# foolwood/SiamMask

Hardware: NVIDIA H100
Metric: search-region frames/sec (127/255 SiamMask-sharp) (higher is better)
Workload: dtype f16x3 (hi+lo split fp16 operands on wgmma, f32 accumulate; f32 CUDA-core xcorr/refine)

## Files before the change

siammask_b200/csrc/common.cuh:

```cuda
#pragma once
#include <cuda.h>
#include <cuda_fp16.h>
#include <cuda_runtime.h>
#include <cstdint>
#include <cstdio>
#include <stdexcept>
#include <string>
#include <vector>

struct sm_image_desc;

namespace smk {

struct Act {
  __half* hi = nullptr;
  __half* lo = nullptr;
  int B = 0, H = 0, W = 0, C = 0;
  int sexp = 0;
  __host__ __device__ size_t numel() const { return (size_t)B * H * W * C; }
  __host__ __device__ int M() const { return B * H * W; }
};

struct ConvGeom {
  int Cin, Cout, KH, KW, stride, pad, dil;
// ... 8 lines not shown
  const __half* res_hi = nullptr;
  const __half* res_lo = nullptr;
  __half* out_hi = nullptr;
  __half* out_lo = nullptr;
  float* out_f32 = nullptr;
  int out_mode = OUT_NHWC_SPLIT;
  int relu = 0;
  int* ovf = nullptr;
};

__device__ __forceinline__ void flag_if_out_of_range(float absmax, int* ovf) {
  if (ovf != nullptr && !(absmax <= 65504.f)) atomicOr(ovf, 1);
}
constexpr int kStatusBadSlot = 2;

struct GemmSegment {
  CUtensorMap tmA[2];
  int kind;
  int mode;
  int num_kb, cblks, KW;
  int stride, pad, dil;
  int b_col0;
};

struct GemmParams {
  GemmSegment seg[2];
  int nseg;
  CUtensorMap tmB[2];
  int M, Cout, Ho, Wo;
  int n_tiles, m_tiles;
  int reverse_m;
  Epilogue ep;
};

struct GemmInput {
  Act in;
  ConvGeom g;
  int w_col0;
};

struct TrackerHp {
  double context_amount, penalty_k, window_influence, lr;
  int32_t exemplar_size, instance_size, total_stride, base_size, out_size, reserved;
};

struct CudaError : std::runtime_error {
  using std::runtime_error::runtime_error;
};

#define SMK_CUDA(expr)                                                                              \
  do {                                                                                              \
    cudaError_t _e = (expr);                                                                        \
    if (_e != cudaSuccess)                                                                          \
      throw smk::CudaError(std::string(#expr) + " failed: " + cudaGetErrorString(_e) + " at " +    \
                           __FILE__ + ":" + std::to_string(__LINE__));                              \
  } while (0)

#define SMK_CHECK(cond, msg)                                                                        \
  do {                                                                                              \
    if (!(cond)) throw std::runtime_error(std::string("check failed: ") + #cond + " — " + (msg));   \
  } while (0)

template <typename K>
inline void ensure_dynamic_smem(K kernel, int bytes, unsigned long long& done_mask) {
  int dev = 0;
  SMK_CUDA(cudaGetDevice(&dev));
  const unsigned long long bit = 1ull << (dev & 63);
  if (done_mask & bit) return;
  SMK_CUDA(cudaFuncSetAttribute(kernel, cudaFuncAttributeMaxDynamicSharedMemorySize, bytes));
  done_mask |= bit;
}


bool gemm_conv_supported(const ConvGeom& g);
void launch_gemm_conv(const Act& in, const ConvGeom& g, const __half* w_hi, const __half* w_lo, int cout_pad,
                      const Epilogue& ep, int nsplit, int num_sms, cudaStream_t st);
void launch_gemm_multi(const GemmInput* convs, int nconv, const Act* residual, int res_col0, const __half* w_hi,
                       const __half* w_lo, int cout_pad, int w_ld, const Epilogue& ep, int nsplit, int num_sms,
                       cudaStream_t st, bool reverse_m = false);

CUtensorMap make_map_tiled_nd(const __half* base, int rank, const uint64_t* dims, const uint64_t* strides_bytes,
                              const uint32_t* box, int swizzle_bytes);

bool patch_conv_supported(const Act& in, const ConvGeom& g);
void launch_conv3x3_patch(const Act& in, const ConvGeom& g, const __half* w_hi, const __half* w_lo, int w_ld,
                          const Epilogue& ep, int nsplit, int num_sms, cudaStream_t st);

void launch_stem_tc(const float* x_nchw, int B, int S, const __half* w_hi, const __half* w_lo, const float* alpha,
                    const float* beta, Act out, int num_sms, cudaStream_t st, int* ovf = nullptr);

void launch_ref_conv(const Act& in, const ConvGeom& g, const float* w_krsc_cout, const Epilogue& ep,
                     cudaStream_t st);
void launch_stem(const float* x_nchw, int B, int S, const float* w, const float* alpha, const float* beta, Act out,
                 cudaStream_t st);
void launch_maxpool3s2(const Act& in, Act out, cudaStream_t st);
void launch_xcorr_nhwc(const Act& x, int c_off, const __half* k_hi, const __half* k_lo, int kh, int kw, Act out,
                       float mul, int* ovf, cudaStream_t st, const int32_t* slots = nullptr, int num_slots = 0);
void launch_scatter_slots(const __half* src_hi, const __half* src_lo, __half* dst_hi, __half* dst_lo,
                          const int32_t* slots, int B, int num_slots, int n, int* status, cudaStream_t st);
void launch_paste_labels(const float* masks, int side, const double* maps, const uint8_t* anno, const int32_t* obj_off,
                         const int32_t* objects, int G, int H, int W, double seg_thr, uint8_t* labels, cudaStream_t st,
                         const sm_image_desc* desc = nullptr);
void launch_paste_labels_iou(const float* masks, int side, const double* maps, const uint8_t* anno,
                             const int32_t* obj_off, const int32_t* objects, const int32_t* target_ids, int G, int H,
                             int W, double seg_thr, uint8_t* labels, const double* thrs, int T, int32_t* counts,
                             cudaStream_t st, const sm_image_desc* desc = nullptr);
void launch_label_boxes(const uint8_t* anno, int G, int H, int W, const int32_t* queries, int Q, int32_t* boxes,
                        cudaStream_t st, const sm_image_desc* desc = nullptr);
void launch_vot_overlap(const float* poly_a, const float* poly_b, int B, int W, int H, float* overlap, cudaStream_t st,
                        const int32_t* wh = nullptr);
void launch_absmax(const Act& a, float* slot, cudaStream_t st);
void launch_xcorr_nchw_f32(const float* x, const float* k, float* out, int planes, int H, int W, int kh, int kw,
                           cudaStream_t st);
int launch_xcorr_bulk_f32(const float* x, const float* k, float* out, int planes, int H, int W, int kh, int kw,
                          cudaStream_t st);
void launch_crop_center(const Act& in, int crop, Act out, cudaStream_t st);
void launch_refine_crop(const Act& in, const int32_t* pos, int pos_max, int scale, int padv, int size, Act out,
                        cudaStream_t st);
void launch_gather_corr(const Act& corr, const int32_t* pos, float* out, float mul, cudaStream_t st);
void launch_gather_mask_col(const float* mask, const int32_t* pos, int B, int C, int R, float* out, cudaStream_t st);
void launch_deconv(const float* p3, const float* w, const float* bias, float* out, int B, int Cin, int N,
                   int cout, cudaStream_t st);
void launch_split_to_f32(const Act& in, float* out, cudaStream_t st, float mul = 1.f);
void launch_import_nchw(const float* x_nchw, Act out, cudaStream_t st);
void launch_warp_affine(const float* src, int sh, int sw, const double* maps, float* dst, int dh, int dw, float border,
                        int B, cudaStream_t st, const sm_image_desc* dst_desc = nullptr);
void launch_tracker_prepare(int B, const double* state, const int32_t* avg, const TrackerHp& hp, int32_t* boxes,
                            double* tsz, double* aux, cudaStream_t st);
void launch_tracker_update(int B, double* state, const float* rec, const double* aux, const int32_t* imsize,
                           const TrackerHp& hp, int A, int R, double* maps, double* out, cudaStream_t st,
                           const double* hp_table = nullptr);
void launch_crop_resize(const uint8_t* frames, size_t frame_stride, int H, int W, const int32_t* box, int B, int model,
                        float* out, cudaStream_t st, const int32_t* frame_idx = nullptr,
                        const sm_image_desc* desc = nullptr);
void launch_select(const float* cls, const float* loc, const float* anchors, const float* window, const double* tsz,
                   int B, int A, int R, double penalty_k, double window_influence, int32_t* best_idx, int32_t* pos,
                   float* rec, cudaStream_t st, const double* hp = nullptr);
void launch_mask_iou(const float* masks, int side, const double* maps, const uint8_t* anno, const int32_t* video, int B,
                     int H, int W, const double* thrs, int T, int32_t* counts, cudaStream_t st);
void launch_small_conv3x3_maps(const float* a, const float* b, int B, int Hi, int Wi, int Ho, int Wo, int Cin, int Cout,
                               const int* ymap, const int* xmap, const float* w, const float* bias, int relu,
                               float* out, cudaStream_t st);
std::vector<int> nearest_index_table(int out_size, int in_size);
int gemm_cout_pad(int cout);

}
```

siammask_b200/csrc/conv3x3_patch_sm90.cu:

```cuda
#include "common.cuh"
#include "ptx.cuh"

#include <cstdlib>

namespace smk {

namespace {

constexpr int P_THREADS = 384;
constexpr int P_CONSUMER_WARPS = 8;
constexpr int P_SLACK_ROWS = 8;

template <int CM, int NSPLIT>
struct PCfg {
  static constexpr int NKB = CM / 64;
  static constexpr int B_TILE_BYTES = CM * 128;
  static constexpr int B_STAGE_BYTES = NSPLIT * B_TILE_BYTES;
  static constexpr int B_STAGES = 3;
  static constexpr int ACC = CM / 2;
};

struct PatchParams {
  CUtensorMap tmA[2];
  CUtensorMap tmB[2];
  int B, H, W, PW, RO;
  int tiles_per_img, num_tiles;
  int panel_bytes;
  int patch_rows;
  Epilogue ep;
};

__device__ __forceinline__ void tma_load_4d(void* dst, const CUtensorMap* map, uint64_t* bar, int c0, int c1, int c2,
                                            int c3) {
  asm volatile(
      "cp.async.bulk.tensor.4d.shared::cluster.global.mbarrier::complete_tx::bytes"
      " [%0], [%1, {%3, %4, %5, %6}], [%2];" ::"r"(smem_u32(dst)),
      "l"(reinterpret_cast<uint64_t>(map)), "r"(smem_u32(bar)), "r"(c0), "r"(c1), "r"(c2), "r"(c3)
      : "memory");
}

template <int CM, int NSPLIT>
__global__ void __launch_bounds__(P_THREADS, 1) conv3x3_patch_kernel(const __grid_constant__ PatchParams p) {
  using C = PCfg<CM, NSPLIT>;
  constexpr int NKB = C::NKB;
  extern __shared__ uint8_t smem_raw[];
  uint8_t* smem = reinterpret_cast<uint8_t*>((reinterpret_cast<uintptr_t>(smem_raw) + 1023) & ~uintptr_t(1023));
  const int patch_bytes = NSPLIT * p.panel_bytes;
  uint8_t* bring = smem + 2 * patch_bytes;
  uint64_t* pfull = reinterpret_cast<uint64_t*>(bring + C::B_STAGES * C::B_STAGE_BYTES);
  uint64_t* pempty = pfull + 2;
  uint64_t* bfull = pempty + 2;
  uint64_t* bempty = bfull + C::B_STAGES;

  const int warp = __shfl_sync(0xffffffffu, (int)(threadIdx.x >> 5), 0), lane = threadIdx.x & 31;
  const int slack_bytes = P_SLACK_ROWS * 128;
  for (int pb = 0; pb < 2 * NSPLIT; ++pb) {
    uint8_t* panel = smem + pb * p.panel_bytes;
    for (int i = threadIdx.x * 16; i < 2 * slack_bytes; i += P_THREADS * 16) {
      uint8_t* dst = i < slack_bytes ? panel + i : panel + slack_bytes + p.patch_rows * 128 + (i - slack_bytes);
      *reinterpret_cast<uint4*>(dst) = make_uint4(0, 0, 0, 0);
    }
  }
  fence_proxy_async();
  if (threadIdx.x == 0) {
    for (int i = 0; i < NSPLIT; ++i) { tma_prefetch_desc(&p.tmA[i]); tma_prefetch_desc(&p.tmB[i]); }
    for (int i = 0; i < 2; ++i) { mbar_init(&pfull[i], 1); mbar_init(&pempty[i], P_CONSUMER_WARPS); }
    for (int i = 0; i < C::B_STAGES; ++i) { mbar_init(&bfull[i], 1); mbar_init(&bempty[i], P_CONSUMER_WARPS); }
    fence_barrier_init();
  }
  __syncthreads();

  if (warp < 4) {
    setmaxnreg_dec<40>();
    if (warp != 0) return;
    const bool leader = elect_one();
    const int my_tiles = (p.num_tiles - (int)blockIdx.x + (int)gridDim.x - 1) / (int)gridDim.x;
    const int units = my_tiles * NKB;
    auto issue_patch = [&](int u) {
      const int tile = blockIdx.x + (u / NKB) * gridDim.x;
      const int kb = u % NKB;
      const int b = tile / p.tiles_per_img;
      const int y0 = (tile - b * p.tiles_per_img) * p.RO;
      const int pbuf = u & 1;
      const uint32_t pph = (u >> 1) & 1;
      mbar_wait(&pempty[pbuf], pph ^ 1);
      if (leader) {
        mbar_arrive_expect_tx(&pfull[pbuf], NSPLIT * p.patch_rows * 128);
#pragma unroll
        for (int s = 0; s < NSPLIT; ++s)
          tma_load_4d(smem + (pbuf * NSPLIT + s) * p.panel_bytes + slack_bytes, &p.tmA[s], &pfull[pbuf], kb * 64, -1,
                      y0 - 1, b);
      }
      __syncwarp();
    };
    int bstage = 0;
    uint32_t bphase = 0;
    if (units > 0) issue_patch(0);
    for (int u = 0; u < units; ++u) {
      const int kb = u % NKB;
      for (int tap = 0; tap < 9; ++tap) {
        if (tap == C::B_STAGES && u + 1 < units) issue_patch(u + 1);
        mbar_wait(&bempty[bstage], bphase ^ 1);
        if (leader) {
          mbar_arrive_expect_tx(&bfull[bstage], C::B_STAGE_BYTES);
          uint8_t* st = bring + bstage * C::B_STAGE_BYTES;
#pragma unroll
          for (int s = 0; s < NSPLIT; ++s)
            tma_load_2d(st + s * C::B_TILE_BYTES, &p.tmB[s], &bfull[bstage], tap * CM + kb * 64, 0);
        }
        __syncwarp();
        if (++bstage == C::B_STAGES) { bstage = 0; bphase ^= 1; }
      }
    }
    return;
  }

  setmaxnreg_inc<232>();
  const int wg = (warp >> 2) - 1;
  const int wl = warp & 3;
  const Epilogue& ep = p.ep;
  float acc[C::ACC];
  float acc2[C::ACC];
  int unit = 0, bstage = 0;
  uint32_t bphase = 0;
  for (int tile = blockIdx.x; tile < p.num_tiles; tile += gridDim.x) {
#pragma unroll
    for (int i = 0; i < C::ACC; ++i) { acc[i] = 0.f; acc2[i] = 0.f; }
    for (int kb = 0; kb < NKB; ++kb, ++unit) {
      const int pbuf = unit & 1;
      const uint32_t pph = (unit >> 1) & 1;
      mbar_wait(&pfull[pbuf], pph);
      const uint32_t a_hi0 = smem_u32(smem + (pbuf * NSPLIT) * p.panel_bytes + slack_bytes) + wg * (64 * 128);
      const uint32_t a_lo0 = a_hi0 + p.panel_bytes;
      int prev = -1;
#pragma unroll 1
      for (int tap = 0; tap < 9; ++tap) {
        const int r = tap / 3, s = tap - 3 * r;
        const int shift = (r * p.PW + s - 1) * 128;
        mbar_wait(&bfull[bstage], bphase);
        const uint32_t b_hi = smem_u32(bring + bstage * C::B_STAGE_BYTES);
        const uint64_t da_hi = wgmma_desc_kmajor<128>(a_hi0 + shift);
        const uint64_t da_lo = wgmma_desc_kmajor<128>(a_lo0 + shift);
        const uint64_t db_hi = wgmma_desc_kmajor<128>(b_hi);
        const uint64_t db_lo = wgmma_desc_kmajor<128>(b_hi + C::B_TILE_BYTES);
        wgmma_fence();
#pragma unroll
        for (int k = 0; k < 4; ++k) {
          const uint64_t kadd = static_cast<uint64_t>(k * 2);
          wgmma_f16<CM>(acc, da_hi + kadd, db_hi + kadd);
          if constexpr (NSPLIT == 2) {
            wgmma_f16<CM>(acc2, da_hi + kadd, db_lo + kadd);
            wgmma_f16<CM>(acc2, da_lo + kadd, db_hi + kadd);
          }
        }
        wgmma_commit();
        wgmma_wait<1>();
        if (prev >= 0) {
          __syncwarp();
          if (lane == 0) mbar_arrive(&bempty[prev]);
        }
        prev = bstage;
        if (++bstage == C::B_STAGES) { bstage = 0; bphase ^= 1; }
      }
      wgmma_wait<0>();
      __syncwarp();
      if (lane == 0) {
        mbar_arrive(&bempty[prev]);
        mbar_arrive(&pempty[pbuf]);
      }
    }
    fence_regs(acc);
    if constexpr (NSPLIT == 2) fence_regs(acc2);

    const int b = tile / p.tiles_per_img;
    const int y0 = (tile - b * p.tiles_per_img) * p.RO;
    const int j0 = wg * 64 + wl * 16 + (lane >> 2);
    float amax = 0.f;
#pragma unroll
    for (int h = 0; h < 2; ++h) {
      const int j = j0 + 8 * h;
      const int yy = j / p.PW, xx = j - yy * p.PW;
      const int y = y0 + yy, x = xx - 1;
      if (!(x >= 0 && x < p.W && y < p.H && yy < p.RO)) continue;
      const size_t off0 = ((static_cast<size_t>(b) * p.H + y) * p.W + x) * CM;
#pragma unroll
      for (int q = 0; q < CM / 8; ++q) {
        const int n = 8 * q + 2 * (lane & 3);
        float v0 = acc[4 * q + 2 * h], v1 = acc[4 * q + 2 * h + 1];
        if constexpr (NSPLIT == 2) {
          v0 += acc2[4 * q + 2 * h];
          v1 += acc2[4 * q + 2 * h + 1];
        }
        const float2 al = __ldg(reinterpret_cast<const float2*>(ep.alpha + n));
        const float2 be = __ldg(reinterpret_cast<const float2*>(ep.beta + n));
        v0 = fmaf(v0, al.x, be.x);
        v1 = fmaf(v1, al.y, be.y);
        if (ep.relu) {
          v0 = fmaxf(v0, 0.f);
          v1 = fmaxf(v1, 0.f);
        }
        amax = fmaxf(amax, fmaxf(fabsf(v0), fabsf(v1)));
        const __half2 hv = __floats2half2_rn(v0, v1);
        const float2 hf = __half22float2(hv);
        *reinterpret_cast<__half2*>(ep.out_hi + off0 + n) = hv;
        if (ep.out_lo != nullptr)
          *reinterpret_cast<__half2*>(ep.out_lo + off0 + n) = __floats2half2_rn(v0 - hf.x, v1 - hf.y);
      }
    }
    flag_if_out_of_range(amax, ep.ovf);
  }
}

int patch_pw(int W) { return (W + 1 + 7) / 8 * 8; }

int patch_ro(int W) {
  const int pw = patch_pw(W);
  return 128 % pw == 0 ? 128 / pw : 0;
}

template <int CM, int NSPLIT>
void launch_patch(const PatchParams& p, int num_sms, cudaStream_t st) {
  using C = PCfg<CM, NSPLIT>;
  const int smem = 2 * NSPLIT * p.panel_bytes + C::B_STAGES * C::B_STAGE_BYTES + 256 + 1024;
  SMK_CHECK(smem <= 227 * 1024, "patch conv: shared memory budget");
  auto kern = conv3x3_patch_kernel<CM, NSPLIT>;
  static unsigned long long attr = 0;
  ensure_dynamic_smem(kern, 227 * 1024, attr);
  const int grid = p.num_tiles < num_sms ? p.num_tiles : num_sms;
  kern<<<grid, P_THREADS, smem, st>>>(p);
  SMK_CUDA(cudaGetLastError());
}

}

bool patch_conv_supported(const Act& in, const ConvGeom& g) {
  if (!(g.KH == 3 && g.KW == 3 && g.stride == 1 && g.pad == 1 && g.dil == 1 && g.Cin == g.Cout)) return false;
  if (!(g.Cin == 64 || g.Cin == 128)) return false;
  if (in.H != in.W) return false;
  return patch_ro(in.W) >= 1 && patch_pw(in.W) <= 64;
}

void launch_conv3x3_patch(const Act& in, const ConvGeom& g, const __half* w_hi, const __half* w_lo, int w_ld,
                          const Epilogue& ep, int nsplit, int num_sms, cudaStream_t st) {
  SMK_CHECK(patch_conv_supported(in, g), "patch conv: unsupported geometry");
  SMK_CHECK(ep.out_mode == OUT_NHWC_SPLIT && ep.res_hi == nullptr, "patch conv writes NHWC split planes, no residual");
  SMK_CHECK(nsplit == 1 || (in.lo != nullptr && w_lo != nullptr && ep.out_lo != nullptr), "exact mode needs lo planes");
  SMK_CHECK(w_ld >= 9 * g.Cin, "weight row length");
  PatchParams p;
  p.B = in.B; p.H = in.H; p.W = in.W;
  p.PW = patch_pw(in.W);
  p.RO = patch_ro(in.W);
  p.tiles_per_img = (in.H + p.RO - 1) / p.RO;
  p.num_tiles = in.B * p.tiles_per_img;
  p.patch_rows = (p.RO + 2) * p.PW;
  p.panel_bytes = (p.patch_rows + 2 * P_SLACK_ROWS) * 128;
  SMK_CHECK(p.panel_bytes % 1024 == 0, "patch panels must keep the 1024-byte swizzle alignment");
  p.ep = ep;
  for (int s = 0; s < nsplit; ++s) {
    const __half* a = s == 0 ? in.hi : in.lo;
    const uint64_t dims[4] = {(uint64_t)in.C, (uint64_t)in.W, (uint64_t)in.H, (uint64_t)in.B};
    const uint64_t strides[3] = {(uint64_t)in.C * 2, (uint64_t)in.W * in.C * 2, (uint64_t)in.H * in.W * in.C * 2};
    const uint32_t box[4] = {64, (uint32_t)p.PW, (uint32_t)(p.RO + 2), 1};
    p.tmA[s] = make_map_tiled_nd(a, 4, dims, strides, box, 128);
    const uint64_t wd[2] = {(uint64_t)w_ld, (uint64_t)g.Cout};
    const uint64_t ws[1] = {(uint64_t)w_ld * 2};
    const uint32_t wb[2] = {64, (uint32_t)g.Cout};
    p.tmB[s] = make_map_tiled_nd(s == 0 ? w_hi : w_lo, 2, wd, ws, wb, 128);
  }
  if (nsplit == 1) { p.tmA[1] = p.tmA[0]; p.tmB[1] = p.tmB[0]; }
  if (g.Cin == 64) {
    if (nsplit == 2) launch_patch<64, 2>(p, num_sms, st); else launch_patch<64, 1>(p, num_sms, st);
  } else {
    if (nsplit == 2) launch_patch<128, 2>(p, num_sms, st); else launch_patch<128, 1>(p, num_sms, st);
  }
}

}
```

siammask_b200/csrc/engine.cu:

```cuda
#include "../../include/siammask_b200.h"
#include "common.cuh"

#include <algorithm>
#include <cmath>
#include <cstdlib>
#include <cstring>
#include <map>
#include <memory>
#include <unordered_map>

namespace smk {

namespace {

constexpr float BN_EPS = 1e-5f;
constexpr size_t ALIGN = 256;
inline size_t align_up(size_t x) { return (x + ALIGN - 1) / ALIGN * ALIGN; }

thread_local std::string g_last_error;

struct ConvW {
  ConvGeom g{};
  int cout_pad = 0;
  bool gemm_ok = false;
// ... 879 lines not shown
        const int step = !(mx[i] <= 65504.f) ? -10 : (mx[i] == 0.f && iter < 8) ? +10 : 0;
        if (step != 0) set_scale(absmax_names_[i], std::max(-60, std::min(60, scale_of(absmax_names_[i]) + step)));
      }
      rewire_and_upload();
      continue;
    }
    settled = true;
    for (size_t i = 0; i < mx.size(); ++i) {
      if (mx[i] == 0.f) continue;
      const int cur = scale_of(absmax_names_[i]);
      if (mx[i] >= 256.f && mx[i] <= 4096.f) continue;
      int want = cur + (int)std::lround(std::log2(1024.0 / (double)mx[i]));
      want = std::max(-60, std::min(60, want));
      const auto it = layers_.find(absmax_names_[i]);
      if (it != layers_.end() && it->second.f32_out) want = 0;
      if (want != cur) { set_scale(absmax_names_[i], want); settled = false; }
    }
    if (!settled) rewire_and_upload();
  }
  SMK_CHECK(settled, "calibrate(): activation scales did not settle (non-finite network outputs?)");
}

int Engine::status() {
  int v = 0;
  SMK_CUDA(cudaDeviceSynchronize());
  SMK_CUDA(cudaMemcpy(&v, ovf_flag_, sizeof(int), cudaMemcpyDeviceToHost));
  return v;
}


Act Engine::alloc_act(Arena& ar, int B, int H, int W, int C) {
  Act a;
  a.B = B; a.H = H; a.W = W; a.C = C;
  a.hi = static_cast<__half*>(ar.alloc(a.numel() * sizeof(__half)));
  a.lo = exact_ ? static_cast<__half*>(ar.alloc(a.numel() * sizeof(__half))) : nullptr;
  return a;
}

F32T Engine::alloc_f32(Arena& ar, int B, int H, int W, int C) {
  F32T t;
  t.B = B; t.H = H; t.W = W; t.C = C;
  t.p = static_cast<float*>(ar.alloc((size_t)B * H * W * C * sizeof(float)));
  return t;
}

void Engine::conv_into(const Act& in, const ConvW& Lw, Epilogue ep, cudaStream_t st, const Act* res,
                       const Act* in2) {
  ep.beta = Lw.beta;
  const double M = (double)in.B * Lw.g.out_size(in.H) * Lw.g.out_size(in.W);
  double K = (double)Lw.g.KH * Lw.g.KW * Lw.g.Cin;
  const bool tc = cfg_.backend == SM_BACKEND_TENSOR && Lw.gemm_ok;
  SMK_CHECK(in2 == nullptr || (tc && Lw.fused2), "fused second input needs the tensor-core path");
  if (in2 != nullptr) K += (double)Lw.g2.KH * Lw.g2.KW * Lw.g2.Cin;
  if (calibrating_) {
    ConvW& W = const_cast<ConvW&>(Lw);
    auto name_of = [&](const Act& a) {
      auto it = tensor_name_.find(a.hi);
      return it == tensor_name_.end() ? std::string() : it->second;
    };
    W.src_in = name_of(in);
    W.src_in2 = in2 ? name_of(*in2) : std::string();
    W.src_res = res ? name_of(*res) : std::string();
    W.f32_out = ep.out_mode != OUT_NHWC_SPLIT;
  }
  SMK_CHECK(in.sexp == Lw.s_in && (in2 == nullptr || in2->sexp == Lw.s_in2) && (res == nullptr || res->sexp == Lw.s_res),
            "activation scale mismatch at " + Lw.conv_key + " (weights were packed for other scales: re-run calibrate)");
  SMK_CHECK(ep.out_mode == OUT_NHWC_SPLIT || Lw.s_out == 0, "fp32 outputs are unscaled");
  if (ep.out_mode == OUT_NHWC_SPLIT) ep.ovf = ovf_flag_;
  const double flops = 2.0 * M * K * Lw.g.Cout;
  const double bytes = 4.0 * ((double)in.numel() + (in2 ? (double)in2->numel() : 0.0) + M * Lw.g.Cout * (res ? 2 : 1) +
                              K * Lw.g.Cout);
  if (!tc) {
    SMK_CHECK(Lw.s_in == 0 && Lw.s_out == 0, "the SIMT backend runs unscaled activations only");
    ep.alpha = ones_;
    if (res != nullptr) { ep.res_hi = res->hi; ep.res_lo = res->lo; }
    launch(st, 1, Lw.conv_key, "conv_simt", flops, bytes, [&] { launch_ref_conv(in, Lw.g, Lw.w_ref, ep, st); });
    return;
  }
  ep.alpha = Lw.alpha;
  const Act* big = &in;
  if (in2 != nullptr && in2->numel() > big->numel()) big = in2;
  if (res != nullptr && res->numel() > big->numel()) big = res;
  const bool use_patch = in2 == nullptr && res == nullptr && ep.out_mode == OUT_NHWC_SPLIT &&
                         patch_conv_supported(in, Lw.g);
  const bool reverse = !use_patch && end_of(*big) > 0;
  GemmInput gi[2] = {{in, Lw.g, 0}, {in, Lw.g, 0}};
  int nconv = 1;
  const Act* ident = nullptr;
  if (in2 != nullptr) {
    gi[1] = {*in2, Lw.g2, Lw.col2};
    nconv = 2;
    ep.beta = Lw.beta2;
  } else if (res != nullptr) {
    if (Lw.has_diag) ident = res;
    else { ep.res_hi = res->hi; ep.res_lo = res->lo; }
  }
  launch(st, 1, Lw.conv_key, "conv_gemm", flops, bytes, [&] {
    const int now_end = reverse ? -1 : +1;
    last_end_[in.hi] = now_end;
    if (in2 != nullptr) last_end_[in2->hi] = now_end;
    if (res != nullptr) last_end_[res->hi] = now_end;
    if (ep.out_mode == OUT_NHWC_SPLIT) last_end_[ep.out_hi] = now_end;
    if (use_patch)
      launch_conv3x3_patch(in, Lw.g, Lw.w_hi, Lw.w_lo, Lw.w_ld, ep, exact_ ? 2 : 1, num_sms_, st);
    else
      launch_gemm_multi(gi, nconv, ident, Lw.col_diag, Lw.w_hi, Lw.w_lo, Lw.cout_pad, Lw.w_ld, ep, exact_ ? 2 : 1,
                        num_sms_, st, reverse);
  });
}

void Engine::note_tensor(const Act& a, const std::string& name, cudaStream_t st, const Act* same_scale_as) {
  if (measuring_) return;
  if (taps_ != nullptr) (*taps_)[name] = a;
  if (!calibrating_) return;
  if (same_scale_as != nullptr) {
    tensor_name_[a.hi] = tensor_name_[same_scale_as->hi];
    return;
  }
  tensor_name_[a.hi] = name;
  size_t slot = 0;
  for (; slot < absmax_names_.size(); ++slot)
    if (absmax_names_[slot] == name) break;
  if (slot == absmax_names_.size()) {
    SMK_CHECK((int)slot < kAbsmaxSlots, "too many calibrated tensors");
    absmax_names_.push_back(name);
  }
  launch_absmax(a, absmax_dev_ + slot, st);
}

void Engine::note_tensor(const F32T& t, const std::string& name) {
  if (!measuring_ && taps_f32_ != nullptr) (*taps_f32_)[name] = t;
}

Act Engine::conv(const Act& in, const ConvW& Lw, bool relu, const Act* res, Arena& ar, cudaStream_t st,
                 const Act* in2) {
  Act out = alloc_act(ar, in.B, Lw.g.out_size(in.H), Lw.g.out_size(in.W), Lw.g.Cout);
  Epilogue ep;
  ep.relu = relu ? 1 : 0;
  ep.out_mode = OUT_NHWC_SPLIT;
  ep.out_hi = out.hi;
  ep.out_lo = out.lo;
  out.sexp = Lw.s_out;
  conv_into(in, Lw, ep, st, res, in2);
  note_tensor(out, Lw.conv_key, st);
  return out;
}

F32T Engine::conv_f32(const Act& in, const ConvW& Lw, bool relu, Arena& ar, cudaStream_t st) {
  F32T out = alloc_f32(ar, in.B, Lw.g.out_size(in.H), Lw.g.out_size(in.W), Lw.g.Cout);
  Epilogue ep;
  ep.relu = relu ? 1 : 0;
  ep.out_mode = OUT_NHWC_F32;
  ep.out_f32 = out.p;
  conv_into(in, Lw, ep, st);
  note_tensor(out, Lw.conv_key);
  return out;
}

Act Engine::backbone(const float* x, int B, int S, Arena& ar, std::map<std::string, Act>* keep, cudaStream_t st) {
  const std::string F = "features.features.";
  const int So = (S - 7) / 2 + 1;
  Act p0 = alloc_act(ar, B, So, So, 64);
  const ConvW& stem = L(F + "conv1");
  launch(st, 1, "stem", "stem", 2.0 * B * So * So * 64 * 147, 4.0 * B * (3.0 * S * S + 64.0 * So * So), [&] {
    if (cfg_.backend == SM_BACKEND_TENSOR)
      launch_stem_tc(x, B, S, stem_whi_, stem_wlo_, stem_alpha_, stem.beta, p0, num_sms_, st, ovf_flag_);
    else launch_stem(x, B, S, stem.w_ref, ones_, stem.beta, p0, st);
// ... 509 lines not shown
  SMK_CUDA(cudaDeviceSynchronize());
  std::string out;
  for (auto& r : prof_) {
    float ms = 0.f;
    cudaEventElapsedTime(&ms, r.e0, r.e1);
    char line[512];
    snprintf(line, sizeof line, "%s\t%s\t%.6f\t%.0f\t%.0f\n", r.name.c_str(), r.cat.c_str(), ms, r.flops, r.bytes);
    out += line;
    event_pool_.push_back(r.e0);
    event_pool_.push_back(r.e1);
  }
  prof_.clear();
  return out;
}


static void conv2d_op(const float* x, const float* w, const float* scale, const float* shift, float* out, int B,
                      int Cin, int H, int W, int Cout, int KH, int KW, int stride, int pad, int dil, int relu,
                      int backend, int precision, cudaStream_t st) {
  ConvGeom g{Cin, Cout, KH, KW, stride, pad, dil};
  const bool exact = precision == SM_PRECISION_EXACT;
  const bool use_gemm = backend == SM_BACKEND_TENSOR;
  SMK_CHECK(!use_gemm || gemm_conv_supported(g), "tensor-core conv needs Cin % 64 == 0");
  const size_t K = (size_t)KH * KW * Cin;
  const int cout_pad = use_gemm ? gemm_cout_pad(Cout) : Cout;
  std::vector<float> hw(K * Cout), hs(Cout, 1.f), hb(Cout, 0.f);
  SMK_CUDA(cudaStreamSynchronize(st));
  SMK_CUDA(cudaMemcpy(hw.data(), w, hw.size() * sizeof(float), cudaMemcpyDeviceToHost));
  if (scale) SMK_CUDA(cudaMemcpy(hs.data(), scale, Cout * sizeof(float), cudaMemcpyDeviceToHost));
  if (shift) SMK_CUDA(cudaMemcpy(hb.data(), shift, Cout * sizeof(float), cudaMemcpyDeviceToHost));
  std::vector<float> wref(K * Cout), alpha(cout_pad, 0.f), beta(cout_pad, 0.f);
  std::vector<__half> whi((size_t)cout_pad * K, __float2half_rn(0.f)), wlo((size_t)cout_pad * K, __float2half_rn(0.f));
  const int HW = KH * KW;
  for (int n = 0; n < Cout; ++n) {
    float amax = 0.f;
    for (int c = 0; c < Cin; ++c)
      for (int t = 0; t < HW; ++t) {
        const float fw = (float)((double)hw[((size_t)n * Cin + c) * HW + t] * (double)hs[n]);
        wref[((size_t)t * Cin + c) * Cout + n] = fw;
        amax = std::max(amax, std::fabs(fw));
      }
    beta[n] = hb[n];
    alpha[n] = 1.f;
    if (use_gemm) {
      const int e = weight_exp(amax);
      alpha[n] = std::ldexp(1.f, -e);
      for (int c = 0; c < Cin; ++c)
        for (int t = 0; t < HW; ++t) {
          const float fw = std::ldexp(wref[((size_t)t * Cin + c) * Cout + n], e);
          const __half h = __float2half_rn(fw);
          whi[((size_t)n * HW + t) * Cin + c] = h;
          wlo[((size_t)n * HW + t) * Cin + c] = __float2half_rn(fw - __half2float(h));
        }
    }
  }
  const int Ho = g.out_size(H), Wo = g.out_size(W);
  Act in;
  in.B = B; in.H = H; in.W = W; in.C = Cin;
  __half *d_whi = nullptr, *d_wlo = nullptr;
  float *d_wref = nullptr, *d_alpha = nullptr, *d_beta = nullptr;
  SMK_CUDA(cudaMalloc(&in.hi, in.numel() * sizeof(__half)));
  if (exact) SMK_CUDA(cudaMalloc(&in.lo, in.numel() * sizeof(__half)));
  SMK_CUDA(cudaMalloc(&d_whi, whi.size() * sizeof(__half)));
  SMK_CUDA(cudaMalloc(&d_wlo, wlo.size() * sizeof(__half)));
  SMK_CUDA(cudaMalloc(&d_wref, wref.size() * sizeof(float)));
  SMK_CUDA(cudaMalloc(&d_alpha, alpha.size() * sizeof(float)));
  SMK_CUDA(cudaMalloc(&d_beta, beta.size() * sizeof(float)));
  SMK_CUDA(cudaMemcpy(d_whi, whi.data(), whi.size() * sizeof(__half), cudaMemcpyHostToDevice));
  SMK_CUDA(cudaMemcpy(d_wlo, wlo.data(), wlo.size() * sizeof(__half), cudaMemcpyHostToDevice));
  SMK_CUDA(cudaMemcpy(d_wref, wref.data(), wref.size() * sizeof(float), cudaMemcpyHostToDevice));
  SMK_CUDA(cudaMemcpy(d_alpha, alpha.data(), alpha.size() * sizeof(float), cudaMemcpyHostToDevice));
  SMK_CUDA(cudaMemcpy(d_beta, beta.data(), beta.size() * sizeof(float), cudaMemcpyHostToDevice));
  launch_import_nchw(x, in, st);
  Epilogue ep;
  ep.alpha = d_alpha;
  ep.beta = d_beta;
  ep.relu = relu;
  ep.out_mode = OUT_NCHW_F32;
  ep.out_f32 = out;
  int dev = 0, sms = 132;
  SMK_CUDA(cudaGetDevice(&dev));
  SMK_CUDA(cudaDeviceGetAttribute(&sms, cudaDevAttrMultiProcessorCount, dev));
  (void)Ho; (void)Wo;
  if (use_gemm && patch_conv_supported(in, g)) {
    Act o;
    o.B = B; o.H = Ho; o.W = Wo; o.C = Cout;
    SMK_CUDA(cudaMalloc(&o.hi, o.numel() * sizeof(__half)));
    if (exact) SMK_CUDA(cudaMalloc(&o.lo, o.numel() * sizeof(__half)));
    Epilogue e2 = ep;
    e2.out_mode = OUT_NHWC_SPLIT;
    e2.out_hi = o.hi;
    e2.out_lo = o.lo;
    e2.out_f32 = nullptr;
    launch_conv3x3_patch(in, g, d_whi, d_wlo, (int)K, e2, exact ? 2 : 1, sms, st);
    launch_split_to_f32(o, out, st);
    SMK_CUDA(cudaStreamSynchronize(st));
    cudaFree(o.hi); cudaFree(o.lo);
  } else if (use_gemm) launch_gemm_conv(in, g, d_whi, d_wlo, cout_pad, ep, exact ? 2 : 1, sms, st);
  else launch_ref_conv(in, g, d_wref, ep, st);
  SMK_CUDA(cudaStreamSynchronize(st));
  cudaFree(in.hi); cudaFree(in.lo); cudaFree(d_whi); cudaFree(d_wlo); cudaFree(d_wref); cudaFree(d_alpha); cudaFree(d_beta);
}

}


struct sm_engine {
  std::unique_ptr<smk::Engine> impl;
};

#define SM_API_BEGIN try {
#define SM_API_END                                  \
  return 0;                                         \
  }                                                 \
  catch (const std::exception& ex) {                \
    smk::g_last_error = ex.what();                  \
    return -1;                                      \
  }                                                 \
  catch (...) {                                     \
    smk::g_last_error = "unknown error";            \
    return -1;                                      \
  }

static void require_device() {
  int ndev = 0;
  SMK_CHECK(cudaGetDeviceCount(&ndev) == cudaSuccess && ndev > 0, "no CUDA device: siammask_b200 has no CPU fallback");
}

extern "C" {

const char* sm_last_error(void) { return smk::g_last_error.c_str(); }
const char* sm_version(void) { return "siammask_b200 0.1 (sm_90a)"; }

int sm_engine_create(const sm_config* cfg, sm_engine** out) {
  SM_API_BEGIN
  SMK_CHECK(cfg != nullptr && out != nullptr, "null argument");
  require_device();
  auto* e = new sm_engine;
  try {
    e->impl.reset(new smk::Engine(*cfg));
  } catch (...) {
    delete e;
    throw;
  }
  *out = e;
  SM_API_END
}

void sm_engine_destroy(sm_engine* e) { delete e; }

int sm_engine_load_weights(sm_engine* e, const sm_tensor_desc* tensors, int32_t n) {
  SM_API_BEGIN
  SMK_CHECK(e && tensors && n > 0, "null argument");
  e->impl->load_weights(tensors, n);
  SM_API_END
}

int sm_engine_weight_blob(sm_engine* e, void** dev_ptr, size_t* bytes) {
  SM_API_BEGIN
  SMK_CHECK(e && dev_ptr && bytes, "null argument");
  e->impl->weight_blob(dev_ptr, bytes);
  SM_API_END
}

int sm_engine_adopt_weights(sm_engine* e) {
  SM_API_BEGIN
  SMK_CHECK(e, "null argument");
// ... 398 lines not shown
```

Before: 3770.

## Generalize 3x3 patch conv to flat 128-row tiles, N-tiling and adaptive stages

The implicit 3x3 patch convolution no longer requires square inputs, Cin==Cout in {64,128}, or widths where 128 is a multiple of the padded row width. It now uses flat 128-pixel M tiles over a W+1 padded row, tiles Cout by 64 or 128 columns, and sizes the weight pipeline depth (up to 4) from the shared-memory budget. The patch buffer for the next K-block is released at the first tap of the following block rather than after a full wgmma drain per K-block, which keeps tensor-core issue overlapped across K-blocks. More SiamMask convolutions can take the TMA/wgmma patch path instead of the generic GEMM, at the cost of some wasted rows from padding and more index arithmetic per tile.

```diff
diff --git a/siammask_b200/csrc/common.cuh b/siammask_b200/csrc/common.cuh
--- a/siammask_b200/csrc/common.cuh
+++ b/siammask_b200/csrc/common.cuh
@@ -114,7 +114,7 @@
 CUtensorMap make_map_tiled_nd(const __half* base, int rank, const uint64_t* dims, const uint64_t* strides_bytes,
                               const uint32_t* box, int swizzle_bytes);
 
-bool patch_conv_supported(const Act& in, const ConvGeom& g);
+bool patch_conv_supported(const Act& in, const ConvGeom& g, int nsplit);
 void launch_conv3x3_patch(const Act& in, const ConvGeom& g, const __half* w_hi, const __half* w_lo, int w_ld,
                           const Epilogue& ep, int nsplit, int num_sms, cudaStream_t st);
 
diff --git a/siammask_b200/csrc/conv3x3_patch_sm90.cu b/siammask_b200/csrc/conv3x3_patch_sm90.cu
--- a/siammask_b200/csrc/conv3x3_patch_sm90.cu
+++ b/siammask_b200/csrc/conv3x3_patch_sm90.cu
@@ -1,6 +1,7 @@
 #include "common.cuh"
 #include "ptx.cuh"
 
+#include <algorithm>
 #include <cstdlib>
 
 namespace smk {
@@ -10,24 +11,32 @@
 constexpr int P_THREADS = 384;
 constexpr int P_CONSUMER_WARPS = 8;
 constexpr int P_SLACK_ROWS = 8;
-
-template <int CM, int NSPLIT>
+constexpr int P_TILE = 128;
+constexpr int P_MAX_STAGES = 4;
+constexpr int P_SMEM_LIMIT = 227 * 1024;
+constexpr int P_SMEM_EXTRA = 1024 + 256;
+
+template <int BN, int NSPLIT>
 struct PCfg {
-  static constexpr int NKB = CM / 64;
-  static constexpr int B_TILE_BYTES = CM * 128;
+  static constexpr int B_TILE_BYTES = BN * 128;
   static constexpr int B_STAGE_BYTES = NSPLIT * B_TILE_BYTES;
-  static constexpr int B_STAGES = 3;
-  static constexpr int ACC = CM / 2;
+  static constexpr int ACC = BN / 2;
 };
 
 struct PatchParams {
   CUtensorMap tmA[2];
   CUtensorMap tmB[2];
-  int B, H, W, PW, RO;
-  int tiles_per_img, num_tiles;
+  int B, H, W, Cout, PW;
+  int cin, nkb;
+  int rows;
+  int tiles_per_img, m_tiles, n_tiles;
   int panel_bytes;
-  int patch_rows;
+  int stages;
   Epilogue ep;
+};
+
+struct PatchPlan {
+  int PW = 0, rows = 0, tiles_per_img = 0, bn = 0, panel_bytes = 0, stages = 0, smem = 0;
 };
 
 __device__ __forceinline__ void tma_load_4d(void* dst, const CUtensorMap* map, uint64_t* bar, int c0, int c1, int c2,
@@ -39,25 +48,35 @@
       : "memory");
 }
 
-template <int CM, int NSPLIT>
+struct PTile {
+  int b, t0, n0;
+};
+__device__ __forceinline__ PTile patch_tile(const PatchParams& p, int tile, int bn) {
+  const int mb = tile / p.n_tiles;
+  const int nt = tile - mb * p.n_tiles;
+  const int b = mb / p.tiles_per_img;
+  return {b, (mb - b * p.tiles_per_img) * P_TILE, nt * bn};
+}
+
+template <int BN, int NSPLIT>
 __global__ void __launch_bounds__(P_THREADS, 1) conv3x3_patch_kernel(const __grid_constant__ PatchParams p) {
-  using C = PCfg<CM, NSPLIT>;
-  constexpr int NKB = C::NKB;
+  using C = PCfg<BN, NSPLIT>;
   extern __shared__ uint8_t smem_raw[];
   uint8_t* smem = reinterpret_cast<uint8_t*>((reinterpret_cast<uintptr_t>(smem_raw) + 1023) & ~uintptr_t(1023));
   const int patch_bytes = NSPLIT * p.panel_bytes;
   uint8_t* bring = smem + 2 * patch_bytes;
-  uint64_t* pfull = reinterpret_cast<uint64_t*>(bring + C::B_STAGES * C::B_STAGE_BYTES);
+  uint64_t* pfull = reinterpret_cast<uint64_t*>(bring + p.stages * C::B_STAGE_BYTES);
   uint64_t* pempty = pfull + 2;
   uint64_t* bfull = pempty + 2;
-  uint64_t* bempty = bfull + C::B_STAGES;
+  uint64_t* bempty = bfull + P_MAX_STAGES;
 
   const int warp = __shfl_sync(0xffffffffu, (int)(threadIdx.x >> 5), 0), lane = threadIdx.x & 31;
   const int slack_bytes = P_SLACK_ROWS * 128;
+  const int patch_rows = p.rows * p.PW;
   for (int pb = 0; pb < 2 * NSPLIT; ++pb) {
     uint8_t* panel = smem + pb * p.panel_bytes;
     for (int i = threadIdx.x * 16; i < 2 * slack_bytes; i += P_THREADS * 16) {
-      uint8_t* dst = i < slack_bytes ? panel + i : panel + slack_bytes + p.patch_rows * 128 + (i - slack_bytes);
+      uint8_t* dst = i < slack_bytes ? panel + i : panel + slack_bytes + patch_rows * 128 + (i - slack_bytes);
       *reinterpret_cast<uint4*>(dst) = make_uint4(0, 0, 0, 0);
     }
   }
@@ -65,31 +84,30 @@
   if (threadIdx.x == 0) {
     for (int i = 0; i < NSPLIT; ++i) { tma_prefetch_desc(&p.tmA[i]); tma_prefetch_desc(&p.tmB[i]); }
     for (int i = 0; i < 2; ++i) { mbar_init(&pfull[i], 1); mbar_init(&pempty[i], P_CONSUMER_WARPS); }
-    for (int i = 0; i < C::B_STAGES; ++i) { mbar_init(&bfull[i], 1); mbar_init(&bempty[i], P_CONSUMER_WARPS); }
+    for (int i = 0; i < p.stages; ++i) { mbar_init(&bfull[i], 1); mbar_init(&bempty[i], P_CONSUMER_WARPS); }
     fence_barrier_init();
   }
   __syncthreads();
+  const int num_tiles = p.m_tiles * p.n_tiles;
 
   if (warp < 4) {
     setmaxnreg_dec<40>();
     if (warp != 0) return;
     const bool leader = elect_one();
-    const int my_tiles = (p.num_tiles - (int)blockIdx.x + (int)gridDim.x - 1) / (int)gridDim.x;
-    const int units = my_tiles * NKB;
+    const int my_tiles = (num_tiles - (int)blockIdx.x + (int)gridDim.x - 1) / (int)gridDim.x;
+    const int units = my_tiles * p.nkb;
     auto issue_patch = [&](int u) {
-      const int tile = blockIdx.x + (u / NKB) * gridDim.x;
-      const int kb = u % NKB;
-      const int b = tile / p.tiles_per_img;
-      const int y0 = (tile - b * p.tiles_per_img) * p.RO;
+      const PTile t = patch_tile(p, blockIdx.x + (u / p.nkb) * gridDim.x, BN);
+      const int kb = u % p.nkb;
       const int pbuf = u & 1;
       const uint32_t pph = (u >> 1) & 1;
       mbar_wait(&pempty[pbuf], pph ^ 1);
       if (leader) {
-        mbar_arrive_expect_tx(&pfull[pbuf], NSPLIT * p.patch_rows * 128);
+        mbar_arrive_expect_tx(&pfull[pbuf], NSPLIT * patch_rows * 128);
 #pragma unroll
         for (int s = 0; s < NSPLIT; ++s)
-          tma_load_4d(smem + (pbuf * NSPLIT + s) * p.panel_bytes + slack_bytes, &p.tmA[s], &pfull[pbuf], kb * 64, -1,
-                      y0 - 1, b);
+          tma_load_4d(smem + (pbuf * NSPLIT + s) * p.panel_bytes + slack_bytes, &p.tmA[s], &pfull[pbuf], kb * 64,
+                      -1, t.t0 / p.PW - 1, t.b);
       }
       __syncwarp();
     };
@@ -97,19 +115,20 @@
     uint32_t bphase = 0;
     if (units > 0) issue_patch(0);
     for (int u = 0; u < units; ++u) {
-      const int kb = u % NKB;
+      const int n0 = patch_tile(p, blockIdx.x + (u / p.nkb) * gridDim.x, BN).n0;
+      const int kb = u % p.nkb;
       for (int tap = 0; tap < 9; ++tap) {
-        if (tap == C::B_STAGES && u + 1 < units) issue_patch(u + 1);
+        if (tap == p.stages && u + 1 < units) issue_patch(u + 1);
         mbar_wait(&bempty[bstage], bphase ^ 1);
         if (leader) {
           mbar_arrive_expect_tx(&bfull[bstage], C::B_STAGE_BYTES);
           uint8_t* st = bring + bstage * C::B_STAGE_BYTES;
 #pragma unroll
           for (int s = 0; s < NSPLIT; ++s)
-            tma_load_2d(st + s * C::B_TILE_BYTES, &p.tmB[s], &bfull[bstage], tap * CM + kb * 64, 0);
+            tma_load_2d(st + s * C::B_TILE_BYTES, &p.tmB[s], &bfull[bstage], tap * p.cin + kb * 64, n0);
         }
         __syncwarp();
-        if (++bstage == C::B_STAGES) { bstage = 0; bphase ^= 1; }
+        if (++bstage == p.stages) { bstage = 0; bphase ^= 1; }
       }
     }
     return;
@@ -123,76 +142,78 @@
   float acc2[C::ACC];
   int unit = 0, bstage = 0;
   uint32_t bphase = 0;
-  for (int tile = blockIdx.x; tile < p.num_tiles; tile += gridDim.x) {
+  for (int tile = blockIdx.x; tile < num_tiles; tile += gridDim.x) {
+    const int t0 = patch_tile(p, tile, BN).t0;
+    const int base = t0 - (t0 / p.PW - 1) * p.PW + wg * 64 + P_SLACK_ROWS;
 #pragma unroll
     for (int i = 0; i < C::ACC; ++i) { acc[i] = 0.f; acc2[i] = 0.f; }
-    for (int kb = 0; kb < NKB; ++kb, ++unit) {
+    int prev = -1;
+    for (int kb = 0; kb < p.nkb; ++kb, ++unit) {
       const int pbuf = unit & 1;
       const uint32_t pph = (unit >> 1) & 1;
       mbar_wait(&pfull[pbuf], pph);
-      const uint32_t a_hi0 = smem_u32(smem + (pbuf * NSPLIT) * p.panel_bytes + slack_bytes) + wg * (64 * 128);
-      const uint32_t a_lo0 = a_hi0 + p.panel_bytes;
-      int prev = -1;
+      const uint32_t a_hi0 = smem_u32(smem + (pbuf * NSPLIT) * p.panel_bytes) + base * 128;
 #pragma unroll 1
       for (int tap = 0; tap < 9; ++tap) {
         const int r = tap / 3, s = tap - 3 * r;
-        const int shift = (r * p.PW + s - 1) * 128;
+        const uint32_t a_hi = a_hi0 + ((r - 1) * p.PW + (s - 1)) * 128;
         mbar_wait(&bfull[bstage], bphase);
         const uint32_t b_hi = smem_u32(bring + bstage * C::B_STAGE_BYTES);
-        const uint64_t da_hi = wgmma_desc_kmajor<128>(a_hi0 + shift);
-        const uint64_t da_lo = wgmma_desc_kmajor<128>(a_lo0 + shift);
+        const uint64_t da_hi = wgmma_desc_kmajor<128>(a_hi);
+        const uint64_t da_lo = wgmma_desc_kmajor<128>(a_hi + p.panel_bytes);
         const uint64_t db_hi = wgmma_desc_kmajor<128>(b_hi);
         const uint64_t db_lo = wgmma_desc_kmajor<128>(b_hi + C::B_TILE_BYTES);
         wgmma_fence();
 #pragma unroll
         for (int k = 0; k < 4; ++k) {
           const uint64_t kadd = static_cast<uint64_t>(k * 2);
-          wgmma_f16<CM>(acc, da_hi + kadd, db_hi + kadd);
+          wgmma_f16<BN>(acc, da_hi + kadd, db_hi + kadd);
           if constexpr (NSPLIT == 2) {
-            wgmma_f16<CM>(acc2, da_hi + kadd, db_lo + kadd);
-            wgmma_f16<CM>(acc2, da_lo + kadd, db_hi + kadd);
+            wgmma_f16<BN>(acc2, da_hi + kadd, db_lo + kadd);
+            wgmma_f16<BN>(acc2, da_lo + kadd, db_hi + kadd);
           }
         }
         wgmma_commit();
         wgmma_wait<1>();
         if (prev >= 0) {
           __syncwarp();
-          if (lane == 0) mbar_arrive(&bempty[prev]);
+          if (lane == 0) {
+            mbar_arrive(&bempty[prev]);
+            if (tap == 0) mbar_arrive(&pempty[pbuf ^ 1]);
+          }
         }
         prev = bstage;
-        if (++bstage == C::B_STAGES) { bstage = 0; bphase ^= 1; }
+        if (++bstage == p.stages) { bstage = 0; bphase ^= 1; }
       }
-      wgmma_wait<0>();
-      __syncwarp();
-      if (lane == 0) {
-        mbar_arrive(&bempty[prev]);
-        mbar_arrive(&pempty[pbuf]);
-      }
-    }
+    }
+    wgmma_wait<0>();
     fence_regs(acc);
     if constexpr (NSPLIT == 2) fence_regs(acc2);
-
-    const int b = tile / p.tiles_per_img;
-    const int y0 = (tile - b * p.tiles_per_img) * p.RO;
-    const int j0 = wg * 64 + wl * 16 + (lane >> 2);
+    __syncwarp();
+    if (lane == 0) {
+      mbar_arrive(&bempty[prev]);
+      mbar_arrive(&pempty[(unit - 1) & 1]);
+    }
+
+    const PTile t = patch_tile(p, tile, BN);
+    const int j0 = t.t0 + wg * 64 + wl * 16 + (lane >> 2);
     float amax = 0.f;
 #pragma unroll
     for (int h = 0; h < 2; ++h) {
       const int j = j0 + 8 * h;
-      const int yy = j / p.PW, xx = j - yy * p.PW;
-      const int y = y0 + yy, x = xx - 1;
-      if (!(x >= 0 && x < p.W && y < p.H && yy < p.RO)) continue;
-      const size_t off0 = ((static_cast<size_t>(b) * p.H + y) * p.W + x) * CM;
-#pragma unroll
-      for (int q = 0; q < CM / 8; ++q) {
+      const int y = j / p.PW, x = j - y * p.PW - 1;
+      if (!(x >= 0 && y < p.H)) continue;
+      const size_t off0 = ((static_cast<size_t>(t.b) * p.H + y) * p.W + x) * p.Cout + t.n0;
+#pragma unroll
+      for (int q = 0; q < BN / 8; ++q) {
         const int n = 8 * q + 2 * (lane & 3);
         float v0 = acc[4 * q + 2 * h], v1 = acc[4 * q + 2 * h + 1];
         if constexpr (NSPLIT == 2) {
           v0 += acc2[4 * q + 2 * h];
           v1 += acc2[4 * q + 2 * h + 1];
         }
-        const float2 al = __ldg(reinterpret_cast<const float2*>(ep.alpha + n));
-        const float2 be = __ldg(reinterpret_cast<const float2*>(ep.beta + n));
+        const float2 al = __ldg(reinterpret_cast<const float2*>(ep.alpha + t.n0 + n));
+        const float2 be = __ldg(reinterpret_cast<const float2*>(ep.beta + t.n0 + n));
         v0 = fmaf(v0, al.x, be.x);
         v1 = fmaf(v1, al.y, be.y);
         if (ep.relu) {
@@ -211,68 +232,82 @@
   }
 }
 
-int patch_pw(int W) { return (W + 1 + 7) / 8 * 8; }
-
-int patch_ro(int W) {
-  const int pw = patch_pw(W);
-  return 128 % pw == 0 ? 128 / pw : 0;
-}
-
-template <int CM, int NSPLIT>
-void launch_patch(const PatchParams& p, int num_sms, cudaStream_t st) {
-  using C = PCfg<CM, NSPLIT>;
-  const int smem = 2 * NSPLIT * p.panel_bytes + C::B_STAGES * C::B_STAGE_BYTES + 256 + 1024;
-  SMK_CHECK(smem <= 227 * 1024, "patch conv: shared memory budget");
-  auto kern = conv3x3_patch_kernel<CM, NSPLIT>;
+PatchPlan plan_patch(const Act& in, const ConvGeom& g, int nsplit) {
+  PatchPlan pl;
+  if (!(g.KH == 3 && g.KW == 3 && g.stride == 1 && g.pad == 1 && g.dil == 1)) return pl;
+  if (!(g.Cin % 64 == 0 && g.Cout % 64 == 0 && in.C == g.Cin)) return pl;
+  pl.PW = in.W + 1;
+  pl.tiles_per_img = (in.H * pl.PW + P_TILE - 1) / P_TILE;
+  int span = 0;
+  for (int i = 0; i < pl.tiles_per_img; ++i) {
+    const int t0 = i * P_TILE;
+    span = std::max(span, (t0 + P_TILE - 1) / pl.PW - t0 / pl.PW);
+  }
+  pl.rows = span + 3;
+  if (pl.PW > 256 || pl.rows > 256) return pl;
+  pl.bn = g.Cout % 128 == 0 ? 128 : 64;
+  pl.panel_bytes = ((pl.rows * pl.PW + 2 * P_SLACK_ROWS) * 128 + 1023) / 1024 * 1024;
+  const int stage_bytes = nsplit * pl.bn * 128;
+  const int patches = 2 * nsplit * pl.panel_bytes;
+  const int stages = std::min(P_MAX_STAGES, (P_SMEM_LIMIT - P_SMEM_EXTRA - patches) / stage_bytes);
+  if (stages < 2) return pl;
+  pl.stages = stages;
+  pl.smem = patches + stages * stage_bytes + P_SMEM_EXTRA;
+  return pl;
+}
+
+template <int BN, int NSPLIT>
+void launch_patch(const PatchParams& p, int smem, int num_sms, cudaStream_t st) {
+  SMK_CHECK(smem <= P_SMEM_LIMIT, "patch conv: shared memory budget");
+  auto kern = conv3x3_patch_kernel<BN, NSPLIT>;
   static unsigned long long attr = 0;
-  ensure_dynamic_smem(kern, 227 * 1024, attr);
-  const int grid = p.num_tiles < num_sms ? p.num_tiles : num_sms;
+  ensure_dynamic_smem(kern, P_SMEM_LIMIT, attr);
+  const int tiles = p.m_tiles * p.n_tiles;
+  const int grid = tiles < num_sms ? tiles : num_sms;
   kern<<<grid, P_THREADS, smem, st>>>(p);
   SMK_CUDA(cudaGetLastError());
 }
 
 }
 
-bool patch_conv_supported(const Act& in, const ConvGeom& g) {
-  if (!(g.KH == 3 && g.KW == 3 && g.stride == 1 && g.pad == 1 && g.dil == 1 && g.Cin == g.Cout)) return false;
-  if (!(g.Cin == 64 || g.Cin == 128)) return false;
-  if (in.H != in.W) return false;
-  return patch_ro(in.W) >= 1 && patch_pw(in.W) <= 64;
-}
+bool patch_conv_supported(const Act& in, const ConvGeom& g, int nsplit) { return plan_patch(in, g, nsplit).stages > 0; }
 
 void launch_conv3x3_patch(const Act& in, const ConvGeom& g, const __half* w_hi, const __half* w_lo, int w_ld,
                           const Epilogue& ep, int nsplit, int num_sms, cudaStream_t st) {
-  SMK_CHECK(patch_conv_supported(in, g), "patch conv: unsupported geometry");
+  const PatchPlan pl = plan_patch(in, g, nsplit);
+  SMK_CHECK(pl.stages > 0, "patch conv: unsupported geometry");
   SMK_CHECK(ep.out_mode == OUT_NHWC_SPLIT && ep.res_hi == nullptr, "patch conv writes NHWC split planes, no residual");
   SMK_CHECK(nsplit == 1 || (in.lo != nullptr && w_lo != nullptr && ep.out_lo != nullptr), "exact mode needs lo planes");
   SMK_CHECK(w_ld >= 9 * g.Cin, "weight row length");
   PatchParams p;
-  p.B = in.B; p.H = in.H; p.W = in.W;
-  p.PW = patch_pw(in.W);
-  p.RO = patch_ro(in.W);
-  p.tiles_per_img = (in.H + p.RO - 1) / p.RO;
-  p.num_tiles = in.B * p.tiles_per_img;
-  p.patch_rows = (p.RO + 2) * p.PW;
-  p.panel_bytes = (p.patch_rows + 2 * P_SLACK_ROWS) * 128;
-  SMK_CHECK(p.panel_bytes % 1024 == 0, "patch panels must keep the 1024-byte swizzle alignment");
+  p.B = in.B; p.H = in.H; p.W = in.W; p.Cout = g.Cout;
+  p.PW = pl.PW;
+  p.cin = g.Cin;
+  p.nkb = g.Cin / 64;
+  p.rows = pl.rows;
+  p.tiles_per_img = pl.tiles_per_img;
+  p.m_tiles = in.B * pl.tiles_per_img;
+  p.n_tiles = g.Cout / pl.bn;
+  p.panel_bytes = pl.panel_bytes;
+  p.stages = pl.stages;
   p.ep = ep;
   for (int s = 0; s < nsplit; ++s) {
     const __half* a = s == 0 ? in.hi : in.lo;
     const uint64_t dims[4] = {(uint64_t)in.C, (uint64_t)in.W, (uint64_t)in.H, (uint64_t)in.B};
     const uint64_t strides[3] = {(uint64_t)in.C * 2, (uint64_t)in.W * in.C * 2, (uint64_t)in.H * in.W * in.C * 2};
-    const uint32_t box[4] = {64, (uint32_t)p.PW, (uint32_t)(p.RO + 2), 1};
+    const uint32_t box[4] = {64, (uint32_t)p.PW, (uint32_t)p.rows, 1};
     p.tmA[s] = make_map_tiled_nd(a, 4, dims, strides, box, 128);
     const uint64_t wd[2] = {(uint64_t)w_ld, (uint64_t)g.Cout};
     const uint64_t ws[1] = {(uint64_t)w_ld * 2};
-    const uint32_t wb[2] = {64, (uint32_t)g.Cout};
+    const uint32_t wb[2] = {64, (uint32_t)pl.bn};
     p.tmB[s] = make_map_tiled_nd(s == 0 ? w_hi : w_lo, 2, wd, ws, wb, 128);
   }
   if (nsplit == 1) { p.tmA[1] = p.tmA[0]; p.tmB[1] = p.tmB[0]; }
-  if (g.Cin == 64) {
-    if (nsplit == 2) launch_patch<64, 2>(p, num_sms, st); else launch_patch<64, 1>(p, num_sms, st);
+  if (pl.bn == 64) {
+    if (nsplit == 2) launch_patch<64, 2>(p, pl.smem, num_sms, st); else launch_patch<64, 1>(p, pl.smem, num_sms, st);
   } else {
-    if (nsplit == 2) launch_patch<128, 2>(p, num_sms, st); else launch_patch<128, 1>(p, num_sms, st);
-  }
-}
-
-}
+    if (nsplit == 2) launch_patch<128, 2>(p, pl.smem, num_sms, st); else launch_patch<128, 1>(p, pl.smem, num_sms, st);
+  }
+}
+
+}
diff --git a/siammask_b200/csrc/engine.cu b/siammask_b200/csrc/engine.cu
--- a/siammask_b200/csrc/engine.cu
+++ b/siammask_b200/csrc/engine.cu
@@ -985,7 +985,7 @@
   if (in2 != nullptr && in2->numel() > big->numel()) big = in2;
   if (res != nullptr && res->numel() > big->numel()) big = res;
   const bool use_patch = in2 == nullptr && res == nullptr && ep.out_mode == OUT_NHWC_SPLIT &&
-                         patch_conv_supported(in, Lw.g);
+                         patch_conv_supported(in, Lw.g, exact_ ? 2 : 1);
   const bool reverse = !use_patch && end_of(*big) > 0;
   GemmInput gi[2] = {{in, Lw.g, 0}, {in, Lw.g, 0}};
   int nconv = 1;
@@ -1661,7 +1661,7 @@
   SMK_CUDA(cudaGetDevice(&dev));
   SMK_CUDA(cudaDeviceGetAttribute(&sms, cudaDevAttrMultiProcessorCount, dev));
   (void)Ho; (void)Wo;
-  if (use_gemm && patch_conv_supported(in, g)) {
+  if (use_gemm && patch_conv_supported(in, g, exact ? 2 : 1)) {
     Act o;
     o.B = B; o.H = Ho; o.W = Wo; o.C = Cout;
     SMK_CUDA(cudaMalloc(&o.hi, o.numel() * sizeof(__half)));
```

New measurement: 3730 (median of 6 runs). -1.1%, worse.
